# Minimap2onGPU/mm2-gb

Measured on AMD Instinct MI355X. Metric: chaining anchor-pairs/s, higher is better.
Workload: dtype int32+f32

## Files before the change

mm2-gb_amd/csrc/chain_kernels.hip:

```cpp
#include <hip/hip_runtime.h>
#include <stdint.h>
#include <limits.h>
#include <algorithm>
#include "chain_dev.h"
#include "wave_scan.h"

namespace mm2gb {

#define WAVE 64

__device__ __forceinline__ int lane_id() { return threadIdx.x & (WAVE - 1); }
__device__ __forceinline__ int bcast(int v, int src_lane) { return __builtin_amdgcn_readlane(v, src_lane); }
__device__ __forceinline__ int first_lane(int v) { return __builtin_amdgcn_readfirstlane(v); }
__device__ __forceinline__ int wave_max_i32_dpp(int v)
{
	v = max(v, __builtin_amdgcn_update_dpp(INT_MIN, v, 0x111, 0xf, 0xf, false));
	v = max(v, __builtin_amdgcn_update_dpp(INT_MIN, v, 0x112, 0xf, 0xf, false));
	v = max(v, __builtin_amdgcn_update_dpp(INT_MIN, v, 0x114, 0xf, 0xf, false));
	v = max(v, __builtin_amdgcn_update_dpp(INT_MIN, v, 0x118, 0xf, 0xf, false));
	v = max(v, __builtin_amdgcn_update_dpp(INT_MIN, v, 0x142, 0xa, 0xf, false));
	v = max(v, __builtin_amdgcn_update_dpp(INT_MIN, v, 0x143, 0xc, 0xf, false));
	return __builtin_amdgcn_readlane(v, WAVE - 1);
}
__device__ __forceinline__ int prev_lane(int v) { return __builtin_amdgcn_update_dpp(v, v, 0x138, 0xf, 0xf, false); }
// ... 540 lines not shown
			} else sc -= (int)(lin + .5f * lg);
		}
		sc_out = sc;
		return ok;
	}
}

struct Target { int x, y, tag, seg, q, st, hi; bool live; };
struct Keep { int idx, x, hi, y, tag, f; };

typedef const int __attribute__((address_space(4))) *scalar_i32_ptr;
typedef const int __attribute__((address_space(3))) *lds_i32_ptr;
__device__ __forceinline__ scalar_i32_ptr as_scalar(const void *p) { return (scalar_i32_ptr)(uintptr_t)p; }

struct SrcGroup { int x[4], y[4], t[4]; };
__device__ __forceinline__ SrcGroup load_group(const DevBatch &b, int j0)
{
	const scalar_i32_ptr sr = as_scalar(b.raw);
	SrcGroup g;
#pragma unroll
	for (int u = 0; u < 4; ++u) { const size_t at = (size_t)(j0 + u) * 4; g.x[u] = sr[at]; g.y[u] = sr[at + 2]; g.t[u] = tag_of((unsigned)sr[at + 3]); }
	return g;
}
template <bool CHECK, bool CLAMP>
__device__ __forceinline__ void sweep_block_lut(int t_st, int tx4, int ty4, int jb, int k_from, const int4 *stage,
                                                const DevParams &P, int &bestv)
{
	const unsigned base = (unsigned)P.lut_base, last_at = base + ((unsigned)P.lut_last << 2), lim4 = (unsigned)P.dq_lim << 2;
	constexpr int G = SWEEP_GROUP;
	for (int kg = k_from & ~(G - 1); kg < WAVE; kg += G) {
		const int j0 = jb + kg;
		int dqm[G], drm[G], pen[G];
		int4 s4[G];
#pragma unroll
		for (int u = 0; u < G; ++u) s4[u] = stage[kg + u];
#pragma unroll
		for (int u = 0; u < G; ++u) {
			dqm[u] = ty4 - s4[u].w; drm[u] = tx4 - s4[u].z;
			const unsigned at = lut_address(drm[u], dqm[u], base);
			pen[u] = *(lds_i32_ptr)(uintptr_t)(CLAMP ? (at < last_at ? at : last_at) : at);
		}
#pragma unroll
		for (int u = 0; u < G; ++u) {
			const int dg = drm[u] < dqm[u] ? drm[u] : dqm[u];
			int v = ((s4[u].y < dg ? s4[u].y : dg) << 5) + s4[u].x;
			asm("" : "+v"(v));
			v += pen[u];
			if (!CHECK) {
				unsigned long long saved;
				asm volatile("s_mov_b64 %[sv], exec\n\tv_cmpx_gt_u32_e32 vcc, %[lim], %[dq]\n\tv_max_i32_e32 %[b], %[v], %[b]\n\ts_mov_b64 exec, %[sv]"
				             : [b] "+v"(bestv), [sv] "=&s"(saved) : [lim] "s"(lim4), [dq] "v"(dqm[u]), [v] "v"(v) : "vcc");
			} else {
				const bool take = ((unsigned)dqm[u] < lim4) & (v > bestv) & (drm[u] != -4) & (j0 + u >= t_st);
				bestv = take ? v : bestv;
			}
		}
	}
}

template <int MODE, bool CHECK>
__device__ __forceinline__ void sweep_block(const DevBatch &b, const Target &T, int jb, int k_from, int sf,
                                            const DevParams &P, const int *lut, int &best, int &arg)
{
	int kg = k_from & ~3;
	SrcGroup nxt = load_group(b, jb + kg);
	for (; kg < WAVE; kg += 4) {
		const SrcGroup g = nxt;
		const int j0 = jb + kg;
		nxt = load_group(b, kg + 4 < WAVE ? j0 + 4 : j0);
#pragma unroll
		for (int u = 0; u < 4; ++u) {
			const int j = j0 + u;
			const int uf = bcast(sf, kg + u);
			int sc;
			bool take = pair_score<MODE>(T.x, T.y, T.seg, g.x[u], g.y[u], g.t[u], P, lut, sc);
			const int cand = sc + uf;
			take = take && cand >= best;
			if (CHECK) take = take && j >= T.st;
			if (take) { best = cand; arg = j; }
		}
	}
}

__device__ __forceinline__ void stage_block_lut(int xs, int ys, int sf, int sq, int4 *stage, bool far = false, int d0 = 0)
{
	const int k = lane_id();
	const int x4 = (int)((unsigned)xs << 2), y4 = (int)((unsigned)ys << 2);
	stage[k] = make_int4(((sf + 1) << 7) + k + 1 - LUT_BIAS + (far ? (sq - 1) << 7 : 0), far ? (int)((unsigned)(x4 - y4 - d0) ^ 0x80000000u) : (sq - 1) * 4, x4, y4);
	__builtin_amdgcn_wave_barrier();
}
__device__ __forceinline__ void stage_block_lut(const DevBatch &b, int jb, int sf, int sq, int4 *stage)
{
	const int js = jb + lane_id();
	stage_block_lut(a_x(b, js), a_y(b, js), sf, sq, stage);
}
struct TileXY { int x, y, st; };
template <bool FAR>
__device__ __forceinline__ void sweep_block_lut_free(int tx4, int ty4, const int4 *stage, const unsigned base, const int d0, int &bestv)
{
	constexpr int G = 4;
	const int td = (int)((unsigned)(tx4 - ty4 - d0) ^ 0x80000000u);
	for (int kg = 0; kg < WAVE; kg += G) {
		int4 s4[G];
		int dqm[G], drm[G], pen[G], v[G];
#pragma unroll
		for (int u = 0; u < G; ++u) {
			if (FAR) { const int2 h = *(const int2*)&stage[kg + u]; s4[u].x = h.x; s4[u].y = h.y; }
			else s4[u] = stage[kg + u];
		}
#pragma unroll
		for (int u = 0; u < G; ++u) {
			if (FAR) pen[u] = *(lds_i32_ptr)(uintptr_t)lut_address(td, s4[u].y, base);
			else {
				dqm[u] = ty4 - s4[u].w; drm[u] = tx4 - s4[u].z;
				pen[u] = *(lds_i32_ptr)(uintptr_t)lut_address(drm[u], dqm[u], base);
			}
		}
#pragma unroll
		for (int u = 0; u < G; ++u) {
			if (FAR) v[u] = s4[u].x + pen[u];
			else {
				const int dg = drm[u] < dqm[u] ? drm[u] : dqm[u];
				v[u] = ((s4[u].y < dg ? s4[u].y : dg) << 5) + s4[u].x;
				asm("" : "+v"(v[u]));
				v[u] += pen[u];
			}
		}
		asm("v_max3_i32 %0, %1, %2, %0" : "+v"(bestv) : "v"(v[0]), "v"(v[1]));
		asm("v_max3_i32 %0, %1, %2, %0" : "+v"(bestv) : "v"(v[2]), "v"(v[3]));
	}
}
__device__ __forceinline__ void sweep_block_lut_edge(int t_st, int tx4, int ty4, int jb, int k_from, const int4 *stage, const DevParams &P, int &bestv, const int k_to = WAVE)
{
	constexpr int G = 4;
	const unsigned base = (unsigned)P.lut_base, lim4 = (unsigned)P.dq_lim << 2;
	int pos = 0x7fffffff;
	asm volatile("" : "+v"(pos));
	for (int kg = k_from & ~(G - 1); kg < k_to; kg += G) {
		int4 s4[G];
		int dqm[G], drm[G], pen[G];
#pragma unroll
		for (int u = 0; u < G; ++u) s4[u] = stage[kg + u];
#pragma unroll
		for (int u = 0; u < G; ++u) {
			dqm[u] = ty4 - s4[u].w; drm[u] = tx4 - s4[u].z;
			pen[u] = *(lds_i32_ptr)(uintptr_t)lut_address(drm[u], dqm[u] & pos, base);
		}
#pragma unroll
		for (int u = 0; u < G; ++u) {
			const int dg = drm[u] < dqm[u] ? drm[u] : dqm[u];
			int v = ((s4[u].y < dg ? s4[u].y : dg) << 5) + s4[u].x;
			asm("" : "+v"(v));
			v += pen[u];
			const int j = jb + kg + u;
			unsigned long long saved;
			asm volatile("s_mov_b64 %[sv], exec\n\tv_cmpx_gt_u32_e32 vcc, %[lim], %[dq]\n\tv_cmpx_ge_i32_e32 vcc, %[j], %[st]\n\tv_max_i32_e32 %[b], %[v], %[b]\n\ts_mov_b64 exec, %[sv]"
			             : [b] "+v"(bestv), [sv] "=&s"(saved) : [lim] "s"(lim4), [dq] "v"(dqm[u]), [st] "v"(t_st), [j] "s"(j), [v] "v"(v) : "vcc");
		}
	}
}
__device__ __forceinline__ void sweep_staged_lut(const TileXY &T, int jb, int k_from, bool no_check, bool free_block, const int4 *stage, const DevParams &P,
                                                 int &best, int &arg, bool far_block = false, int d0 = 0)
{
	const int tx4 = (int)(((unsigned)T.x - 1u) << 2), ty4 = (int)(((unsigned)T.y - 1u) << 2);
	int bestv = best << 7;
	if (far_block) sweep_block_lut_free<true>(tx4, ty4, stage, (unsigned)P.lut_base, d0, bestv);
	else if (free_block) sweep_block_lut_free<false>(tx4, ty4, stage, (unsigned)P.lut_base, 0, bestv);
	else if (!no_check && !P.lut_clamp) sweep_block_lut_edge(T.st, tx4, ty4, jb, k_from, stage, P, bestv);
	else if (P.lut_clamp) {
		if (no_check) sweep_block_lut<false, true>(T.st, tx4, ty4, jb, k_from, stage, P, bestv);
		else sweep_block_lut<true, true>(T.st, tx4, ty4, jb, k_from, stage, P, bestv);
	} else {
// ... 499 lines not shown
				const int k_from = tile_lo > jb ? tile_lo - jb : 0;
				sweep_any<MODE>(b, T, jb, k_from, sf, sq, jb >= st_hi && jb + WAVE <= eq_lo, stage, P, lut, best, arg);
				sf = nf; sq = nq;
			}
		}
		in_tile<MODE, TRACK>(b, T, i0, n_here, P, lut, stage, best, arg, keep, [&](int jj) { return b.f[jj]; });
		if (T.live) {
			const int i = i0 + lane;
			b.f[i] = arg < 0 ? T.q : best;
			b.p[i] = arg < 0 ? 0 : i - arg;
		}
	}
}

struct TilePair {
	TileXY A, B;
	int n_a, n_b;
	int lo_a, hi_a, lo_b, hi_b;
	int x_first, x_last_a, x_last;
	int best_a, arg_a, best_b, arg_b;
};

__device__ __forceinline__ TileXY load_xy(const DevBatch &b, int i0, int ce, int &best)
{
	const int i = i0 + lane_id();
	const bool live = i < ce;
	const int il = live ? i : ce - 1;
	TileXY t;
	t.x = a_x(b, il); t.y = a_y(b, il);
	t.st = live ? b.st[il] : INT_MAX;
	best = a_span(b, il) + 1;
	return t;
}

__device__ __forceinline__ TilePair load_pair(const DevBatch &b, int i0, int ce)
{
	TilePair t;
	t.n_a = min(WAVE, ce - i0);
	t.n_b = max(0, min(WAVE, ce - i0 - WAVE));
	t.A = load_xy(b, i0, ce, t.best_a);
	t.B = load_xy(b, t.n_b ? i0 + WAVE : i0, ce, t.best_b);
	t.lo_a = first_lane(t.A.st); t.hi_a = bcast(t.A.st, t.n_a - 1);
	t.lo_b = t.n_b ? first_lane(t.B.st) : INT_MAX; t.hi_b = t.n_b ? bcast(t.B.st, t.n_b - 1) : INT_MAX;
	t.x_first = first_lane(t.A.x); t.x_last_a = bcast(t.A.x, t.n_a - 1);
	t.x_last = t.n_b ? bcast(t.B.x, t.n_b - 1) : t.x_last_a;
	t.arg_a = -1; t.arg_b = -1;
	return t;
}

__device__ __forceinline__ void sweep_pair_block(const DevBatch &b, TilePair &t, int jb, int eq_lo, int sf, int sq, int4 *stage, const DevParams &P)
{
	const bool nc_a = jb >= t.hi_a && jb + WAVE <= eq_lo;
	const bool use_b = t.n_b > 0 && jb + WAVE > t.lo_b;
	const bool nc_b = use_b && jb >= t.hi_b && jb + WAVE <= eq_lo;
	const int xs = a_x(b, jb + lane_id()), ys = a_y(b, jb + lane_id());
	const unsigned free_span = (unsigned)(P.dq_lim - P.bw);
	const bool free_block = P.free_sweep && (unsigned)(t.x_last - first_lane(xs)) <= free_span;
	const bool free_a = P.free_sweep && (unsigned)(t.x_last_a - first_lane(xs)) <= free_span;
	const bool single = t.n_b == 0;
	const bool far_block = free_block && nc_a && (nc_b || single) && t.x_first > bcast(xs, WAVE - 1) && __ballot(sq + P.bw > t.x_first - bcast(xs, WAVE - 1)) == 0;
	const int d0 = (first_lane(xs) - first_lane(ys)) * 4;
	stage_block_lut(xs, ys, sf, sq, stage, far_block, d0);
	if (nc_a && nc_b) sweep_staged_lut2(t.A, t.B, jb, free_block, far_block, d0, stage, P, t.best_a, t.arg_a, t.best_b, t.arg_b);
	else {
		sweep_staged_lut(t.A, jb, t.lo_a > jb ? t.lo_a - jb : 0, nc_a, nc_a && free_a, stage, P, t.best_a, t.arg_a, far_block, d0);
		if (use_b) sweep_staged_lut(t.B, jb, t.lo_b > jb ? t.lo_b - jb : 0, nc_b, nc_b && free_block, stage, P, t.best_b, t.arg_b);
	}
	__builtin_amdgcn_wave_barrier();
}

__device__ __forceinline__ void sweep_a_into_b(const DevBatch &b, TilePair &t, int cs, int i0, int f_a, int q_a, int4 *stage, const DevParams &P)
{
	if (i0 + WAVE <= t.lo_b) return;
	stage_block_lut(b, i0, f_a, q_a, stage);
	const int eq_lo = equal_x_run_start(b, cs, i0 + WAVE, first_lane(t.B.x));
	const bool no_check = i0 >= t.hi_b && i0 + WAVE <= eq_lo;
	const bool span_ab = P.free_sweep && (unsigned)(t.x_last - t.x_first) <= (unsigned)(P.dq_lim - P.bw);
	sweep_staged_lut(t.B, i0, t.lo_b > i0 ? t.lo_b - i0 : 0, no_check, no_check && span_ab, stage, P, t.best_b, t.arg_b);
	__builtin_amdgcn_wave_barrier();
}

__device__ __forceinline__ int wave_min_i32(int v) { return -wave_max_i32_dpp(-v); }

__device__ __forceinline__ void sweep_block_lut_band(int t_st, int tx4, int ty4, int idx, const int4 *stage, const DevParams &P, int &bestv)
{
	constexpr int G = 4;
	const unsigned base = (unsigned)P.lut_base, lim4 = (unsigned)P.dq_lim << 2;
	int pos = 0x7fffffff;
	asm volatile("" : "+v"(pos));
	for (int kg = 0; kg < WAVE; kg += G) {
		int4 s4[G];
		int dqm[G], drm[G], pen[G];
#pragma unroll
		for (int u = 0; u < G; ++u) s4[u] = stage[kg + u];
#pragma unroll
		for (int u = 0; u < G; ++u) {
			dqm[u] = ty4 - s4[u].w; drm[u] = tx4 - s4[u].z;
			pen[u] = *(lds_i32_ptr)(uintptr_t)lut_address(drm[u], dqm[u] & pos, base);
		}
#pragma unroll
		for (int u = 0; u < G; ++u) {
			const int dg = drm[u] < dqm[u] ? drm[u] : dqm[u];
			int v = ((s4[u].y < dg ? s4[u].y : dg) << 5) + s4[u].x;
			asm("" : "+v"(v));
			v += pen[u];
			const int j = __builtin_amdgcn_readlane(idx, kg + u);
			unsigned long long saved;
			asm volatile("s_mov_b64 %[sv], exec\n\tv_cmpx_gt_u32_e32 vcc, %[lim], %[dq]\n\tv_cmpx_ge_i32_e32 vcc, %[j], %[st]\n\tv_max_i32_e32 %[b], %[v], %[b]\n\ts_mov_b64 exec, %[sv]"
			             : [b] "+v"(bestv), [sv] "=&s"(saved) : [lim] "s"(lim4), [dq] "v"(dqm[u]), [st] "v"(t_st), [j] "s"(j), [v] "v"(v) : "vcc");
		}
	}
}

__device__ __forceinline__ int band_group(const DevBatch &b, const DevParams &P, int4 *stage, const int tgt, const int jl)
{
	const int lane = lane_id();
	const int l0 = __builtin_ctzll(__ballot(tgt >= 0));
	const int t = tgt >= 0 ? tgt : bcast(tgt, l0);
	const int x = a_x(b, t), y = a_y(b, t), st = b.st[t];
	int best = a_span(b, t) + 1, arg = -1;
	const int lo = wave_min_i32(st), hi_st = wave_max_i32_dpp(st);
	if (lo < jl) {
		const int d = x - y;
		const int dmin = wave_min_i32(d), dmax = wave_max_i32_dpp(d);
		const int gx_min = wave_min_i32(x), gx_max = wave_max_i32_dpp(x);
		const int band_lo = dmin - P.bw;
		const unsigned width = (unsigned)(dmax - dmin) + 2u * (unsigned)P.bw;
		const int tx4 = (int)(((unsigned)x - 1u) << 2), ty4 = (int)(((unsigned)y - 1u) << 2);
		const unsigned free_span = (unsigned)(P.dq_lim - P.bw);
		auto sweep = [&](const int idx) __attribute__((always_inline)) {
			const int xs = a_x(b, idx), ys = a_y(b, idx), sq = a_span(b, idx), sf = b.f[idx];
			const int sx_min = wave_min_i32(xs), sx_max = wave_max_i32_dpp(xs);
			const bool no_check = first_lane(idx) >= hi_st && gx_min > sx_max;
			const bool free_block = no_check && P.free_sweep && (unsigned)(gx_max - sx_min) <= free_span;
			const bool far_block = free_block && __ballot(sq + P.bw > gx_min - xs) == 0;
			const int d0 = (first_lane(xs) - first_lane(ys)) * 4;
			stage_block_lut(xs, ys, sf, sq, stage, far_block, d0);
			int bestv = best << 7;
			if (far_block) sweep_block_lut_free<true>(tx4, ty4, stage, (unsigned)P.lut_base, d0, bestv);
			else if (free_block) sweep_block_lut_free<false>(tx4, ty4, stage, (unsigned)P.lut_base, 0, bestv);
			else if (no_check) sweep_block_lut<false, false>(st, tx4, ty4, 0, 0, stage, P, bestv);
			else sweep_block_lut_band(st, tx4, ty4, idx, stage, P, bestv);
			const int won = bestv & 127;
			const int wj = __shfl(idx, (won - 1) & (WAVE - 1));
			arg = (unsigned)(won - 1) < (unsigned)WAVE ? wj : arg;
			best = bestv >> 7;
			__builtin_amdgcn_wave_barrier();
		};
		int sidx = 0, n_st = 0;
		int jb = lo;
		int dn = jb + lane < jl ? __hip_atomic_load(b.diag + jb + lane, __ATOMIC_RELAXED, __HIP_MEMORY_SCOPE_AGENT) : 0;
		for (; jb < jl; jb += WAVE) {
			const int j = jb + lane;
			const int dj = dn;
			dn = j + WAVE < jl ? __hip_atomic_load(b.diag + j + WAVE, __ATOMIC_RELAXED, __HIP_MEMORY_SCOPE_AGENT) : 0;
			const bool hit = j < jl && (unsigned)(dj - band_lo) <= width;
			const unsigned long long m = __ballot(hit);
			if (m == 0) continue;
			const int c = __popcll(m);
			const int rank = __builtin_amdgcn_mbcnt_hi((unsigned)(m >> 32), __builtin_amdgcn_mbcnt_lo((unsigned)m, 0u));
			const int dst = (hit ? n_st + rank : n_st + c) & (WAVE - 1);
			const int recv = __builtin_amdgcn_ds_permute(dst << 2, j);
			if (n_st + c < WAVE) {
				sidx = lane >= n_st && lane < n_st + c ? recv : sidx;
				n_st += c;
			} else {
				sweep(lane >= n_st ? recv : sidx);
				n_st += c - WAVE;
				sidx = recv;
			}
		}
		if (n_st > 0) sweep(lane < n_st ? sidx : bcast(sidx, n_st - 1));
	}
	if (tgt >= 0) { b.band_res[2 * tgt] = best; b.band_res[2 * tgt + 1] = arg; }
	return lo < jl;
}

__device__ __forceinline__ int band_slab_part(const DevBatch &b, const DevParams &P, int4 *stage, const int s0, const int n, const int jl,
                                              const int g_from, const int g_to)
{
	constexpr int R = 8;
	const int lane = lane_id();
	unsigned key[R];
	int lo = INT_MAX, hi = INT_MIN, st_lo = INT_MAX;
#pragma unroll
	for (int r = 0; r < R; ++r) {
		const int e = r * WAVE + lane;
		const int d = e < n ? a_x(b, s0 + e) - a_y(b, s0 + e) : 0;
		if (e < n) { lo = min(lo, d); hi = max(hi, d); st_lo = min(st_lo, b.st[s0 + e]); }
	}
	if (wave_min_i32(st_lo) >= jl) return 0;
	const int dmin = wave_min_i32(lo), dmax = wave_max_i32_dpp(hi);
	const unsigned range = (unsigned)(dmax - dmin);
	if (range <= 2u * (unsigned)P.bw) {
#pragma unroll
		for (int r = 0; r < R; ++r) key[r] = r * WAVE + lane < n ? (unsigned)(r * WAVE + lane) : ~0u;
	} else {
		const int sh = (range >> 22) ? 32 - __clz((int)(range >> 22)) : 0;
#pragma unroll
		for (int r = 0; r < R; ++r) {
			const int e = r * WAVE + lane;
			key[r] = e < n ? (((unsigned)(a_x(b, s0 + e) - a_y(b, s0 + e) - dmin) >> sh) << 9) | (unsigned)e : ~0u;
		}
#pragma unroll
		for (int k = 2; k <= R * WAVE; k <<= 1) {
#pragma unroll
			for (int j = k >> 1; j > 0; j >>= 1) {
				if (j >= WAVE) {
					const int jr = j / WAVE;
#pragma unroll
					for (int r = 0; r < R; ++r) {
						if (r & jr) continue;
						const bool up = ((r * WAVE) & k) == 0;
						const unsigned a = key[r], c = key[r | jr];
						key[r] = up ? min(a, c) : max(a, c);
						key[r | jr] = up ? max(a, c) : min(a, c);
					}
				} else {
#pragma unroll
					for (int r = 0; r < R; ++r) {
						const unsigned o = (unsigned)__shfl_xor((int)key[r], j);
						const bool up = ((r * WAVE + lane) & k) == 0, lower = (lane & j) == 0;
						key[r] = up == lower ? min(key[r], o) : max(key[r], o);
					}
				}
			}
		}
	}
	int swept = 0;
	for (int g = g_from; g < g_to; ++g) {
		unsigned kg = key[0];
#pragma unroll
		for (int r = 1; r < R; ++r) kg = g == r ? key[r] : kg;
		const int tgt = kg == ~0u ? -1 : s0 + (int)(kg & 511u);
		if (__ballot(tgt >= 0) == 0) break;
		swept += band_group(b, P, stage, tgt, jl);
	}
	return swept;
}
__device__ __forceinline__ bool band_fits_team(const DevParams &P, const int anchors_per_part, const int n_waves)
{
	return P.band_slab > 0 && P.band_slab / anchors_per_part <= n_waves;
}
__device__ __forceinline__ bool band_chunk(const DevBatch &b, const DevParams &P, const int ci, const int cs, const int ce)
{
	const long long len = ce - cs;
	return P.band_slab > 0 && b.band_res && 2 * (b.chunk_cost[ci] - 16 * len) > (long long)P.band_lag * len;
}

__device__ __forceinline__ void band_merge(const DevBatch &b, const int i0, const int n_here, int &best, int &arg)
{
	const int i = i0 + min(lane_id(), n_here - 1);
	const int bb = __hip_atomic_load(b.band_res + 2 * i, __ATOMIC_RELAXED, __HIP_MEMORY_SCOPE_AGENT);
	const int ba = __hip_atomic_load(b.band_res + 2 * i + 1, __ATOMIC_RELAXED, __HIP_MEMORY_SCOPE_AGENT);
	const bool take = ba >= 0 && (arg < 0 || bb > best);
	best = take ? bb : best;
	arg = take ? ba : arg;
}

__device__ __forceinline__ void band_store_diag(const DevBatch &b, const TilePair &t, const int i0)
{
	if (lane_id() < t.n_a) b.diag[i0 + lane_id()] = t.A.x - t.A.y;
	if (lane_id() < t.n_b) b.diag[i0 + WAVE + lane_id()] = t.B.x - t.B.y;
}

template <bool TRACK>
__device__ __forceinline__ void run_chunk_pairs(const DevBatch &b, const DevParams &P, const int *lut, int4 *stage, const int cs, const int ce, const bool band_on)
{
	const int lane = lane_id();
	Keep keep; keep.idx = -1; keep.x = keep.hi = keep.y = keep.tag = keep.f = 0;
	auto f_old = [&](int jj) { return b.f[jj]; };
	const bool band = band_on;
	int band_groups = 0;
	for (int i0 = cs; i0 < ce; i0 += 2 * WAVE) {
		TilePair t = load_pair(b, i0, ce);
		int jb = cs + ((t.lo_a - cs) & ~(WAVE - 1));
		const int s0 = band ? i0 - (i0 - cs) % P.band_slab : cs, jl = s0 - P.band_lag;
		const bool in_band = band && jl > cs;
		if (band) band_store_diag(b, t, i0);
		if (in_band && i0 == s0) {
			band_groups += band_slab_part(b, P, stage, s0, min(P.band_slab, ce - s0), jl, 0, P.band_slab / WAVE);
			asm volatile("s_waitcnt vmcnt(0)" ::: "memory");
		}
		if (in_band && jb < jl) jb = jl;
		if (jb < i0) {
			const int eq_lo = equal_x_run_start(b, cs, i0, first_lane(t.A.x));
			int sf = b.f[jb + lane], sq = a_span(b, jb + lane);
			for (; jb < i0; jb += WAVE) {
				const int jn = jb + WAVE < i0 ? jb + WAVE + lane : jb + lane;
				const int nf = b.f[jn], nq = a_span(b, jn);
				sweep_pair_block(b, t, jb, eq_lo, sf, sq, stage, P);
				sf = nf; sq = nq;
			}
		}
		const Target TA = load_target(b, i0, ce, TRACK);
		if (in_band && t.lo_a < jl) band_merge(b, i0, t.n_a, t.best_a, t.arg_a);
		in_tile<MODE_LUT, TRACK>(b, TA, i0, t.n_a, P, lut, stage, t.best_a, t.arg_a, keep, f_old);
		const int f_a = t.arg_a < 0 ? TA.q : t.best_a;
		if (TA.live) {
			const int i = i0 + lane;
			b.f[i] = f_a;
			b.p[i] = t.arg_a < 0 ? 0 : i - t.arg_a;
		}
		if (t.n_b == 0) break;
		sweep_a_into_b(b, t, cs, i0, f_a, TA.q, stage, P);
		const Target TB = load_target(b, i0 + WAVE, ce, TRACK);
		if (in_band && t.lo_b < jl) band_merge(b, i0 + WAVE, t.n_b, t.best_b, t.arg_b);
		in_tile<MODE_LUT, TRACK>(b, TB, i0 + WAVE, t.n_b, P, lut, stage, t.best_b, t.arg_b, keep, f_old);
		if (TB.live) {
			const int i = i0 + WAVE + lane;
			b.f[i] = t.arg_b < 0 ? TB.q : t.best_b;
			b.p[i] = t.arg_b < 0 ? 0 : i - t.arg_b;
		}
	}
	if (band_groups > 0 && lane == 0) atomicAdd(&b.counters[CNT_BAND_WAVE], band_groups);
}

struct CoopShared { int done; int keep[6]; int chunk; int bar_count; int bar_gen; int part; int band; };
#define MM2GB_AGENT __HIP_MEMORY_SCOPE_AGENT
__device__ __forceinline__ int  gload(const int *p) { return __hip_atomic_load(p, __ATOMIC_RELAXED, MM2GB_AGENT); }
__device__ __forceinline__ void gstore(int *p, int v) { __hip_atomic_store(p, v, __ATOMIC_RELAXED, MM2GB_AGENT); }
__device__ __forceinline__ void drain_stores() { asm volatile("s_waitcnt vmcnt(0)" ::: "memory"); }
constexpr int SMALL_TEAM = 4, N_SMALL_TEAMS = SCORE_THREADS / WAVE / SMALL_TEAM;
constexpr int N_TEAM_RECORDS = N_SMALL_TEAMS + 3;
constexpr int TAB_INTS = 12;

__device__ __forceinline__ void team_barrier(CoopShared *sh, int team_size)
{
	__builtin_amdgcn_fence(__ATOMIC_RELEASE, "workgroup");
	if (lane_id() == 0) {
		const int gen = __hip_atomic_load(&sh->bar_gen, __ATOMIC_RELAXED, __HIP_MEMORY_SCOPE_WORKGROUP);
		if (__hip_atomic_fetch_add(&sh->bar_count, 1, __ATOMIC_ACQ_REL, __HIP_MEMORY_SCOPE_WORKGROUP) == team_size - 1) {
			__hip_atomic_store(&sh->bar_count, 0, __ATOMIC_RELAXED, __HIP_MEMORY_SCOPE_WORKGROUP);
			__hip_atomic_fetch_add(&sh->bar_gen, 1, __ATOMIC_RELEASE, __HIP_MEMORY_SCOPE_WORKGROUP);
		} else {
			while (__hip_atomic_load(&sh->bar_gen, __ATOMIC_ACQUIRE, __HIP_MEMORY_SCOPE_WORKGROUP) == gen) __builtin_amdgcn_s_sleep(2);
		}
	}
	__builtin_amdgcn_fence(__ATOMIC_ACQUIRE, "workgroup");
}

template <class TT, class SF, class WQ>
__device__ __forceinline__ void sweep_block_by_quarters(const DevBatch &b, const TT &T, const int jb, const int k_from, const int sq, int4 *stage, const DevParams &P,
                                                        int &best, int &arg, SF &&sf_of, WQ &&wait_q)
{
	const int xs = a_x(b, jb + lane_id()), ys = a_y(b, jb + lane_id());
	const int tx4 = (int)(((unsigned)T.x - 1u) << 2), ty4 = (int)(((unsigned)T.y - 1u) << 2);
	for (int q = 0; q < 4; ++q) {
		wait_q(q);
		const int lo = max(k_from, 16 * q), hi = 16 * q + 16;
		if (lo >= hi) continue;
		stage_block_lut(xs, ys, sf_of(), sq, stage);
		int bestv = best << 7;
		sweep_block_lut_edge(T.st, tx4, ty4, jb, lo, stage, P, bestv, hi);
		const int won = bestv & 127;
		arg = (unsigned)(won - 1) < (unsigned)WAVE ? jb + won - 1 : arg;
		best = bestv >> 7;
		__builtin_amdgcn_wave_barrier();
	}
}

template <int MODE, bool TRACK>
__device__ __forceinline__ void coop_chunk(const DevBatch &b, const DevParams &P, const int *lut, int4 *stage, int *ring, const int n_slots, CoopShared *sh,
                           const int cs, const int ce, const int wave, const int n_waves, const bool band_on)
{
	const int lane = lane_id();
	const int n_tiles = (ce - cs + WAVE - 1) / WAVE;
	auto wait_done = [&](int need) {
		while (first_lane(__hip_atomic_load(&sh->done, __ATOMIC_ACQUIRE, __HIP_MEMORY_SCOPE_WORKGROUP)) < need) __builtin_amdgcn_s_sleep(MM2GB_POLL_SLEEP);
	};
	const bool band = MODE == MODE_LUT && band_on && band_fits_team(P, WAVE, n_waves);
	const int tps = band ? P.band_slab / WAVE : 1, s_first = band ? P.band_lag / P.band_slab + 1 : 0;
	int band_groups = 0;
	for (int t = wave; t < n_tiles; t += n_waves) {
		const int i0 = cs + t * WAVE;
		const Target T = load_target(b, i0, ce, TRACK);
		const int n_here = min(WAVE, ce - i0);
		int best = T.q + 1, arg = -1;
		const int tile_lo = first_lane(T.st);
		const int st_hi = bcast(T.st, n_here - 1);
		int jb = cs + ((tile_lo - cs) & ~(WAVE - 1));
		const int sl = t / tps, s0 = cs + sl * P.band_slab, jl = s0 - P.band_lag;
		const bool in_band = band && jl > cs;
		int *band_cnt = sl & 1 ? &sh->band : &sh->part;
		if (band && T.live) b.diag[i0 + lane] = T.x - T.y;
		if (in_band) {
			const int part = t - sl * tps;
			wait_done((jl - cs) / WAVE);
			band_groups += band_slab_part(b, P, stage, s0, min(P.band_slab, ce - s0), jl, part, part + 1);
			if (lane == 0) __hip_atomic_fetch_add(band_cnt, 1, __ATOMIC_RELEASE, __HIP_MEMORY_SCOPE_WORKGROUP);
			if (jb < jl) jb = jl;
		}
		const int eq_lo = MODE == MODE_LUT && jb < i0 ? equal_x_run_start(b, cs, i0, first_lane(T.x)) : i0;
		int slot = (int)((unsigned)((jb - cs) / WAVE) % (unsigned)n_slots);
		for (; jb < i0; jb += WAVE) {
			const int sq = MODE == MODE_LUT ? a_span(b, jb + lane) : 0;
			const int k = (jb - cs) / WAVE, k_from = tile_lo > jb ? tile_lo - jb : 0;
			wait_done(k + 1);
			const int sf = ring[slot * WAVE + lane];
			slot = slot + 1 == n_slots ? 0 : slot + 1;
			sweep_any<MODE>(b, T, jb, k_from, sf, sq, jb >= st_hi && jb + WAVE <= eq_lo, stage, P, lut, best, arg);
		}
		const int my_slot = (int)((unsigned)t % (unsigned)n_slots);
		wait_done(t);
		if (in_band && tile_lo < jl) {
			const int s_min = s_first + ((sl - s_first) & 1);
			const int need = tps * ((sl - s_min) / 2) + min(tps, n_tiles - sl * tps);
			while (first_lane(__hip_atomic_load(band_cnt, __ATOMIC_ACQUIRE, __HIP_MEMORY_SCOPE_WORKGROUP)) < need) __builtin_amdgcn_s_sleep(MM2GB_POLL_SLEEP);
			band_merge(b, i0, n_here, best, arg);
		}
		Keep keep;
		if (TRACK) { keep.idx = first_lane(sh->keep[0]); keep.x = first_lane(sh->keep[1]); keep.hi = first_lane(sh->keep[2]); keep.y = first_lane(sh->keep[3]); keep.tag = first_lane(sh->keep[4]); keep.f = first_lane(sh->keep[5]); }
		else { keep.idx = -1; keep.x = keep.hi = keep.y = keep.tag = keep.f = 0; }
		in_tile<MODE, TRACK>(b, T, i0, n_here, P, lut, stage, best, arg, keep,
		                     [&](int jj) { const unsigned d = (unsigned)(jj - cs); return ring[(d / WAVE) % (unsigned)n_slots * WAVE + d % WAVE]; });
		const int i = i0 + lane;
		const int fi = arg < 0 ? T.q : best;
		if (T.live) {
			ring[my_slot * WAVE + lane] = fi;
			b.f[i] = fi;
			b.p[i] = arg < 0 ? 0 : i - arg;
		}
		if (TRACK && lane == 0) { sh->keep[0] = keep.idx; sh->keep[1] = keep.x; sh->keep[2] = keep.hi; sh->keep[3] = keep.y; sh->keep[4] = keep.tag; sh->keep[5] = keep.f; }
		if (lane == 0) __hip_atomic_store(&sh->done, t + 1, __ATOMIC_RELEASE, __HIP_MEMORY_SCOPE_WORKGROUP);
	}
	if (band_groups > 0 && lane == 0) atomicAdd(&b.counters[CNT_BAND_TEAM], band_groups);
}

template <bool TRACK>
__device__ __forceinline__ void coop_chunk_pairs(const DevBatch &b, const DevParams &P, const int *lut, int4 *stage, int *ring, const int n_slots, CoopShared *sh,
                                 const int cs, const int ce, const int wave, const int n_waves, const bool band_on)
{
	const int lane = lane_id();
	const int n_tiles = (ce - cs + WAVE - 1) / WAVE;
	auto wait_done = [&](int need) {
		while (first_lane(__hip_atomic_load(&sh->done, __ATOMIC_ACQUIRE, __HIP_MEMORY_SCOPE_WORKGROUP)) < need) __builtin_amdgcn_s_sleep(MM2GB_POLL_SLEEP);
	};
	int cur = 0;
	const lds_i32_ptr ring_l = (lds_i32_ptr)(uintptr_t)(unsigned)(uintptr_t)ring;
	auto f_old = [&](int jj) {
		const unsigned d = (unsigned)(jj - cs);
		const int k = (int)(d / WAVE);
		return k >= cur - n_slots ? ring_l[(unsigned)k % (unsigned)n_slots * WAVE + d % WAVE] : b.f[jj];
	};
	const bool band = band_on && band_fits_team(P, 2 * WAVE, n_waves);
	const int pps = band ? P.band_slab / (2 * WAVE) : 1, n_pairs = (n_tiles + 1) / 2, s_first = band ? P.band_lag / P.band_slab + 1 : 0;
	int band_groups = 0;
	for (int pr = wave; 2 * pr < n_tiles; pr += n_waves) {
		const int ta = 2 * pr, i0 = cs + ta * WAVE;
		TilePair t = load_pair(b, i0, ce);
		int jb = cs + ((t.lo_a - cs) & ~(WAVE - 1));
		const int sl = pr / pps, s0 = cs + sl * P.band_slab, jl = s0 - P.band_lag;
		const bool in_band = band && jl > cs;
		int *band_cnt = sl & 1 ? &sh->band : &sh->part;
		if (band) band_store_diag(b, t, i0);
		if (in_band) {
			const int part = pr - sl * pps;
			wait_done((jl - cs) / WAVE);
			band_groups += band_slab_part(b, P, stage, s0, min(P.band_slab, ce - s0), jl, 2 * part, 2 * part + 2);
			if (lane == 0) __hip_atomic_fetch_add(band_cnt, 1, __ATOMIC_RELEASE, __HIP_MEMORY_SCOPE_WORKGROUP);
			if (jb < jl) jb = jl;
		}
		const int eq_lo = jb < i0 ? equal_x_run_start(b, cs, i0, first_lane(t.A.x)) : i0;
		int slot = (int)((unsigned)((jb - cs) / WAVE) % (unsigned)n_slots);
		const int first_in_ring = ta - n_slots;
		int nf = 0;
		if (jb < i0 && (jb - cs) / WAVE < first_in_ring) { wait_done((jb - cs) / WAVE + 1); nf = b.f[jb + lane]; }
		for (; jb < i0; jb += WAVE) {
			const int sq = a_span(b, jb + lane);
			const int k = (jb - cs) / WAVE;
			wait_done(k + 1);
			int sf;
			if (k < first_in_ring) {
				sf = nf;
				if (k + 1 < first_in_ring) { wait_done(k + 2); nf = b.f[jb + WAVE + lane]; }
			} else sf = ring[slot * WAVE + lane];
			slot = slot + 1 == n_slots ? 0 : slot + 1;
			sweep_pair_block(b, t, jb, eq_lo, sf, sq, stage, P);
		}
		const int slot_a = (int)((unsigned)ta % (unsigned)n_slots), slot_b = slot_a + 1 == n_slots ? 0 : slot_a + 1;
		wait_done(ta);
		Keep keep;
		if (TRACK) { keep.idx = first_lane(sh->keep[0]); keep.x = first_lane(sh->keep[1]); keep.hi = first_lane(sh->keep[2]); keep.y = first_lane(sh->keep[3]); keep.tag = first_lane(sh->keep[4]); keep.f = first_lane(sh->keep[5]); }
		else { keep.idx = -1; keep.x = keep.hi = keep.y = keep.tag = keep.f = 0; }
		const Target TA = load_target(b, i0, ce, TRACK);
		if (in_band && t.lo_a < jl) {
			const int s_min = s_first + ((sl - s_first) & 1);
			const int need = pps * ((sl - s_min) / 2) + min(pps, n_pairs - sl * pps);
			while (first_lane(__hip_atomic_load(band_cnt, __ATOMIC_ACQUIRE, __HIP_MEMORY_SCOPE_WORKGROUP)) < need) __builtin_amdgcn_s_sleep(MM2GB_POLL_SLEEP);
			band_merge(b, i0, t.n_a, t.best_a, t.arg_a);
		}
		cur = ta;
		in_tile<MODE_LUT, TRACK>(b, TA, i0, t.n_a, P, lut, stage, t.best_a, t.arg_a, keep, f_old);
		__builtin_amdgcn_s_setprio(MM2GB_INTILE_PRIO);
		const int f_a = t.arg_a < 0 ? TA.q : t.best_a;
		if (TA.live) {
			const int i = i0 + lane;
			ring[slot_a * WAVE + lane] = f_a;
			b.f[i] = f_a;
			b.p[i] = t.arg_a < 0 ? 0 : i - t.arg_a;
		}
		if (t.n_b > 0) {
			if (lane == 0) __hip_atomic_store(&sh->done, ta + 1, __ATOMIC_RELEASE, __HIP_MEMORY_SCOPE_WORKGROUP);
			sweep_a_into_b(b, t, cs, i0, f_a, TA.q, stage, P);
			const Target TB = load_target(b, i0 + WAVE, ce, TRACK);
			if (in_band && t.lo_b < jl) {
				const int s_min = s_first + ((sl - s_first) & 1);
				const int need = pps * ((sl - s_min) / 2) + min(pps, n_pairs - sl * pps);
				while (first_lane(__hip_atomic_load(band_cnt, __ATOMIC_ACQUIRE, __HIP_MEMORY_SCOPE_WORKGROUP)) < need) __builtin_amdgcn_s_sleep(MM2GB_POLL_SLEEP);
				band_merge(b, i0 + WAVE, t.n_b, t.best_b, t.arg_b);
			}
			cur = ta + 1;
			in_tile<MODE_LUT, TRACK>(b, TB, i0 + WAVE, t.n_b, P, lut, stage, t.best_b, t.arg_b, keep, f_old);
			__builtin_amdgcn_s_setprio(MM2GB_INTILE_PRIO);
			if (TB.live) {
				const int i = i0 + WAVE + lane;
				const int f_b = t.arg_b < 0 ? TB.q : t.best_b;
				ring[slot_b * WAVE + lane] = f_b;
				b.f[i] = f_b;
				b.p[i] = t.arg_b < 0 ? 0 : i - t.arg_b;
			}
		}
		if (TRACK && lane == 0) { sh->keep[0] = keep.idx; sh->keep[1] = keep.x; sh->keep[2] = keep.hi; sh->keep[3] = keep.y; sh->keep[4] = keep.tag; sh->keep[5] = keep.f; }
		if (lane == 0) __hip_atomic_store(&sh->done, ta + (t.n_b > 0 ? 2 : 1), __ATOMIC_RELEASE, __HIP_MEMORY_SCOPE_WORKGROUP);
		__builtin_amdgcn_s_setprio(0);
	}
	if (band_groups > 0 && lane == 0) atomicAdd(&b.counters[CNT_BAND_TEAM], band_groups);
}


template <bool TRACK>
__device__ __forceinline__ void gang_chunk_pairs(const DevBatch &b, const DevParams &P, const int *lut, int4 *stage, int *ring, const int n_slots, CoopShared *sh,
                                 GangSlot *gs, int *tab, int &seq, const int cs, const int ce, const int wave)
{
	const int lane = lane_id();
	const int n_tiles = (ce - cs + WAVE - 1) / WAVE;
	const int tpu = first_lane(gload(&gs->tiles_per_wave)) == 2 ? 2 : 1;
	const int STRIP_TILES = tpu * GANG_STRIP_PAIRS;
	int known = 0, known_global = 0;
	auto look_global = [&]() { known_global = max(known_global, first_lane(gload(&gs->done))); known = max(known, known_global); };
	auto wait_done = [&](int need) {
		if (known >= need) return;
		for (;;) {
			known = max(known, first_lane(__hip_atomic_load(&sh->done, __ATOMIC_ACQUIRE, __HIP_MEMORY_SCOPE_WORKGROUP)));
			if (known >= need) return;
// ... 437 lines not shown
```

profiles/isa_loops.py:

```python
#!/usr/bin/env python3
import collections, os, re, subprocess, sys, tempfile
ROOT = os.path.dirname(os.path.dirname(os.path.abspath(__file__)))
SRC = os.path.join(ROOT, "mm2-gb_amd", "csrc", os.environ.get("MM2GB_ISA_SRC", "chain_kernels.hip"))
want = sys.argv[1] if len(sys.argv) > 1 else "k_scoreILi0ELb0ELb0E"
min_len = int(sys.argv[2]) if len(sys.argv) > 2 else 6
HALF = re.compile(r"^v_(sad_u32|min3|max3|lshl_add|add3|and_or|min_|max_|cmp|cmpx|readlane|readfirstlane|writelane|cvt_|mul_lo|mul_hi|mad_|bfe|perm|lshl_or|or3|xad|add_lshl|med3)")

with tempfile.TemporaryDirectory() as td:
    asm = os.path.join(td, "k.s")
    subprocess.run(["/opt/rocm/bin/hipcc", "--offload-arch=gfx950", "-O3", "-std=c++17", "-fPIC", "-ffp-contract=off", "-gline-tables-only", "-I" + os.path.join(ROOT, "include"),
                    "--cuda-device-only", "-S", SRC, "-o", asm], check=True, stderr=subprocess.DEVNULL)
    lines = open(asm).read().splitlines()

src = open(SRC).read().splitlines()
fn_at = []
for i, ln in enumerate(src, 1):
    m = re.match(r"^(?:template\s*<[^>]*>\s*)?(?:static\s+)?(?:__device__|__global__)[^()]*?\b([A-Za-z_][A-Za-z0-9_]*)\s*\(", ln)
    if m:
        fn_at.append((i, m.group(1)))
    else:
        m = re.match(r"^\s+__device__ __forceinline__ [^()]*?\b([A-Za-z_][A-Za-z0-9_]*)\s*\(", ln)
        if m:
            fn_at.append((i, m.group(1)))


def fn_of(line):
    name = "?"
    for at, n in fn_at:
        if at <= line:
            name = n
        else:
            break
    return name


start = next(i for i, ln in enumerate(lines) if ln.startswith("_ZN5mm2gb") and want in ln and ln.rstrip().split(":")[0].endswith(ln.split(":")[0]) and ":" in ln)
end = next(i for i in range(start, len(lines)) if lines[i].startswith(".Lfunc_end"))
file_ids = {}
for ln in lines:
    m = re.match(r'\s*\.file\s+(\d+)\s+"([^"]*)"(?:\s+"([^"]*)")?', ln)
    if m:
        file_ids[int(m.group(1))] = (m.group(3) or m.group(2))
body = []
labels = {}
cur = (0, False)
for i in range(start + 1, end):
    ln = lines[i]
    m = re.match(r"\s*\.loc\s+(\d+)\s+(\d+)", ln)
    if m:
        cur = (int(m.group(2)), file_ids.get(int(m.group(1)), "").endswith(os.path.basename(SRC)))
        continue
    m = re.match(r"^(\.LBB\d+_\d+):", ln)
    if m:
        labels[m.group(1)] = len(body)
        continue
    t = ln.strip()
    if not t or t.startswith(";") or t.startswith("."):
        continue
    body.append((t.split()[0], t, cur[0] if cur[1] else 0))

reg_users = collections.defaultdict(set)
for op, text, _ in body:
    for r in re.findall(r"\bv(\d+)\b", text):
        reg_users[int(r)].add(op)
spill_vgprs = {r for r, ops in reg_users.items() if "v_writelane_b32" in ops and ops <= {"v_writelane_b32", "v_readlane_b32"}}


def is_spill(o):
    if "Spill" in o[1] or "Reload" in o[1] or o[0].startswith("scratch_"):
        return True
    if o[0] == "v_writelane_b32":
        m = re.match(r"v_writelane_b32 v(\d+)", o[1]); return bool(m) and int(m.group(1)) in spill_vgprs
    if o[0] == "v_readlane_b32":
        m = re.match(r"v_readlane_b32 s\d+, v(\d+)", o[1]); return bool(m) and int(m.group(1)) in spill_vgprs
    return False


def mix(ops):
    valu = [o for o in ops if o[0].startswith("v_") and not is_spill(o)]
    return {"n": len(ops), "valu": len(valu), "half": sum(1 for o in valu if HALF.match(o[0])),
            "salu": sum(1 for o in ops if o[0].startswith("s_") and not o[0].startswith(("s_waitcnt", "s_nop"))),
            "lds": sum(1 for o in ops if o[0].startswith("ds_")), "mem": sum(1 for o in ops if o[0].startswith(("global_", "buffer_", "flat_"))),
            "wait": sum(1 for o in ops if o[0].startswith("s_waitcnt")), "spill": sum(1 for o in ops if is_spill(o)),
            "bread": sum(1 for o in ops if o[0] in ("ds_read_b128", "ds_read2_b64", "ds_read_b64") )}


fn_ranges = []
# ... 52 lines not shown
```

Before: 7008 billion.

## Outline band slab pass into noinline function with address-space-typed uniform arguments

Turns band_slab_part into a __noinline__ function. Its arguments are raw address_space(1)/(3) pointers plus scalar params, re-made uniform with readfirstlane. The sweep lambda is folded into a single while loop, the diag key is reused instead of reloading x/y, and the band pass now runs before the tile loads in each driver loop. The aim is to cut register pressure and spills in the main scoring loops by keeping the band code's registers separate. In exchange it adds call overhead and changes the ordering of the band pass relative to the diag stores.

Measured after the change: 7245 billion, median of 6. 3.4% higher.

```diff
diff --git a/mm2-gb_amd/csrc/chain_kernels.hip b/mm2-gb_amd/csrc/chain_kernels.hip
--- a/mm2-gb_amd/csrc/chain_kernels.hip
+++ b/mm2-gb_amd/csrc/chain_kernels.hip
@@ -646,12 +646,15 @@
 	}
 }
 
-__device__ __forceinline__ void stage_block_lut(int xs, int ys, int sf, int sq, int4 *stage, bool far = false, int d0 = 0)
-{
-	const int k = lane_id();
+__device__ __forceinline__ void stage_block_lut_at(const int k, int xs, int ys, int sf, int sq, int4 *stage, bool far = false, int d0 = 0)
+{
 	const int x4 = (int)((unsigned)xs << 2), y4 = (int)((unsigned)ys << 2);
 	stage[k] = make_int4(((sf + 1) << 7) + k + 1 - LUT_BIAS + (far ? (sq - 1) << 7 : 0), far ? (int)((unsigned)(x4 - y4 - d0) ^ 0x80000000u) : (sq - 1) * 4, x4, y4);
 	__builtin_amdgcn_wave_barrier();
+}
+__device__ __forceinline__ void stage_block_lut(int xs, int ys, int sf, int sq, int4 *stage, bool far = false, int d0 = 0)
+{
+	stage_block_lut_at(lane_id(), xs, ys, sf, sq, stage, far, d0);
 }
 __device__ __forceinline__ void stage_block_lut(const DevBatch &b, int jb, int sf, int sq, int4 *stage)
 {
@@ -1317,6 +1320,20 @@
 
 __device__ __forceinline__ int wave_min_i32(int v) { return -wave_max_i32_dpp(-v); }
 
+typedef const int __attribute__((address_space(1))) *glb_i32_cptr;
+typedef int __attribute__((address_space(1))) *glb_i32_ptr;
+typedef int4 __attribute__((address_space(3))) *lds_i32x4_ptr;
+__device__ __forceinline__ int lane_by_count() { return (int)__builtin_amdgcn_mbcnt_hi(~0u, __builtin_amdgcn_mbcnt_lo(~0u, 0u)); }
+struct BandParams { int bw, dq_lim, lut_base, free_sweep, band_slab; };
+template <class T> __device__ __forceinline__ T uniform_glb(T p)
+{
+	const unsigned long long v = (unsigned long long)(uintptr_t)p;
+	return (T)(uintptr_t)(((unsigned long long)(unsigned)first_lane((int)(v >> 32)) << 32) | (unsigned)first_lane((int)v));
+}
+__device__ __forceinline__ int r_x(glb_i32_cptr raw, int i) { return raw[(size_t)i * 4]; }
+__device__ __forceinline__ int r_y(glb_i32_cptr raw, int i) { return raw[(size_t)i * 4 + 2]; }
+__device__ __forceinline__ int r_span(glb_i32_cptr raw, int i) { return (int)((unsigned)raw[(size_t)i * 4 + 3] & 0xffu); }
+
 __device__ __forceinline__ void sweep_block_lut_band(int t_st, int tx4, int ty4, int idx, const int4 *stage, const DevParams &P, int &bestv)
 {
 	constexpr int G = 4;
@@ -1347,13 +1364,15 @@
 	}
 }
 
-__device__ __forceinline__ int band_group(const DevBatch &b, const DevParams &P, int4 *stage, const int tgt, const int jl)
-{
-	const int lane = lane_id();
+struct BandIO { glb_i32_cptr raw, st, f, diag; glb_i32_ptr res; };
+
+__device__ __forceinline__ int band_group(const BandIO &b, const DevParams &P, int4 *stage, const int tgt, const int jl)
+{
+	const int lane = lane_by_count();
 	const int l0 = __builtin_ctzll(__ballot(tgt >= 0));
 	const int t = tgt >= 0 ? tgt : bcast(tgt, l0);
-	const int x = a_x(b, t), y = a_y(b, t), st = b.st[t];
-	int best = a_span(b, t) + 1, arg = -1;
+	const int x = r_x(b.raw, t), y = r_y(b.raw, t), st = b.st[t];
+	int best = r_span(b.raw, t) + 1, arg = -1;
 	const int lo = wave_min_i32(st), hi_st = wave_max_i32_dpp(st);
 	if (lo < jl) {
 		const int d = x - y;
@@ -1363,14 +1382,42 @@
 		const unsigned width = (unsigned)(dmax - dmin) + 2u * (unsigned)P.bw;
 		const int tx4 = (int)(((unsigned)x - 1u) << 2), ty4 = (int)(((unsigned)y - 1u) << 2);
 		const unsigned free_span = (unsigned)(P.dq_lim - P.bw);
-		auto sweep = [&](const int idx) __attribute__((always_inline)) {
-			const int xs = a_x(b, idx), ys = a_y(b, idx), sq = a_span(b, idx), sf = b.f[idx];
+		int sidx = 0, n_st = 0;
+		int jb = lo;
+		int dn = jb + lane < jl ? __hip_atomic_load(b.diag + jb + lane, __ATOMIC_RELAXED, __HIP_MEMORY_SCOPE_AGENT) : 0;
+		while (true) {
+			int idx, carry = 0, n_next = 0;
+			if (jb < jl) {
+				const int j = jb + lane;
+				const int dj = dn;
+				dn = j + WAVE < jl ? __hip_atomic_load(b.diag + j + WAVE, __ATOMIC_RELAXED, __HIP_MEMORY_SCOPE_AGENT) : 0;
+				jb += WAVE;
+				const bool hit = j < jl && (unsigned)(dj - band_lo) <= width;
+				const unsigned long long m = __ballot(hit);
+				if (m == 0) continue;
+				const int c = __popcll(m);
+				const int rank = __builtin_amdgcn_mbcnt_hi((unsigned)(m >> 32), __builtin_amdgcn_mbcnt_lo((unsigned)m, 0u));
+				const int dst = (hit ? n_st + rank : n_st + c) & (WAVE - 1);
+				const int recv = __builtin_amdgcn_ds_permute(dst << 2, j);
+				if (n_st + c < WAVE) {
+					sidx = lane >= n_st && lane < n_st + c ? recv : sidx;
+					n_st += c;
+					continue;
+				}
+				idx = lane >= n_st ? recv : sidx;
+				n_next = n_st + c - WAVE;
+				carry = recv;
+			} else {
+				if (n_st == 0) break;
+				idx = lane < n_st ? sidx : bcast(sidx, n_st - 1);
+			}
+			const int xs = r_x(b.raw, idx), ys = r_y(b.raw, idx), sq = r_span(b.raw, idx), sf = b.f[idx];
 			const int sx_min = wave_min_i32(xs), sx_max = wave_max_i32_dpp(xs);
 			const bool no_check = first_lane(idx) >= hi_st && gx_min > sx_max;
 			const bool free_block = no_check && P.free_sweep && (unsigned)(gx_max - sx_min) <= free_span;
 			const bool far_block = free_block && __ballot(sq + P.bw > gx_min - xs) == 0;
 			const int d0 = (first_lane(xs) - first_lane(ys)) * 4;
-			stage_block_lut(xs, ys, sf, sq, stage, far_block, d0);
+			stage_block_lut_at(lane, xs, ys, sf, sq, stage, far_block, d0);
 			int bestv = best << 7;
 			if (far_block) sweep_block_lut_free<true>(tx4, ty4, stage, (unsigned)P.lut_base, d0, bestv);
 			else if (free_block) sweep_block_lut_free<false>(tx4, ty4, stage, (unsigned)P.lut_base, 0, bestv);
@@ -1381,47 +1428,31 @@
 			arg = (unsigned)(won - 1) < (unsigned)WAVE ? wj : arg;
 			best = bestv >> 7;
 			__builtin_amdgcn_wave_barrier();
-		};
-		int sidx = 0, n_st = 0;
-		int jb = lo;
-		int dn = jb + lane < jl ? __hip_atomic_load(b.diag + jb + lane, __ATOMIC_RELAXED, __HIP_MEMORY_SCOPE_AGENT) : 0;
-		for (; jb < jl; jb += WAVE) {
-			const int j = jb + lane;
-			const int dj = dn;
-			dn = j + WAVE < jl ? __hip_atomic_load(b.diag + j + WAVE, __ATOMIC_RELAXED, __HIP_MEMORY_SCOPE_AGENT) : 0;
-			const bool hit = j < jl && (unsigned)(dj - band_lo) <= width;
-			const unsigned long long m = __ballot(hit);
-			if (m == 0) continue;
-			const int c = __popcll(m);
-			const int rank = __builtin_amdgcn_mbcnt_hi((unsigned)(m >> 32), __builtin_amdgcn_mbcnt_lo((unsigned)m, 0u));
-			const int dst = (hit ? n_st + rank : n_st + c) & (WAVE - 1);
-			const int recv = __builtin_amdgcn_ds_permute(dst << 2, j);
-			if (n_st + c < WAVE) {
-				sidx = lane >= n_st && lane < n_st + c ? recv : sidx;
-				n_st += c;
-			} else {
-				sweep(lane >= n_st ? recv : sidx);
-				n_st += c - WAVE;
-				sidx = recv;
-			}
-		}
-		if (n_st > 0) sweep(lane < n_st ? sidx : bcast(sidx, n_st - 1));
-	}
-	if (tgt >= 0) { b.band_res[2 * tgt] = best; b.band_res[2 * tgt + 1] = arg; }
+			sidx = carry; n_st = n_next;
+		}
+	}
+	if (tgt >= 0) { b.res[2 * tgt] = best; b.res[2 * tgt + 1] = arg; }
 	return lo < jl;
 }
 
-__device__ __forceinline__ int band_slab_part(const DevBatch &b, const DevParams &P, int4 *stage, const int s0, const int n, const int jl,
-                                              const int g_from, const int g_to)
+__device__ __noinline__ int band_slab_part(const glb_i32_cptr raw_, const glb_i32_cptr st_, const glb_i32_cptr f_, const glb_i32_cptr diag_, const glb_i32_ptr res_,
+                                           const BandParams bp, const lds_i32x4_ptr stage_, const int s0_, const int ce_, const int jl_, const int g_from_, const int g_to_)
 {
 	constexpr int R = 8;
-	const int lane = lane_id();
+	const BandIO b = { uniform_glb(raw_), uniform_glb(st_), uniform_glb(f_), uniform_glb(diag_), uniform_glb(res_) };
+	DevParams P = {};
+	P.bw = first_lane(bp.bw); P.dq_lim = first_lane(bp.dq_lim); P.lut_base = first_lane(bp.lut_base); P.free_sweep = first_lane(bp.free_sweep);
+	int4 *stage = (int4*)(lds_i32x4_ptr)(uintptr_t)(unsigned)first_lane((int)(unsigned)(uintptr_t)stage_);
+	const int s0 = first_lane(s0_), jl = first_lane(jl_), g_from = first_lane(g_from_), g_to = first_lane(g_to_);
+	const int n = min(first_lane(bp.band_slab), first_lane(ce_) - s0);
+	const int lane = lane_by_count();
 	unsigned key[R];
 	int lo = INT_MAX, hi = INT_MIN, st_lo = INT_MAX;
 #pragma unroll
 	for (int r = 0; r < R; ++r) {
 		const int e = r * WAVE + lane;
-		const int d = e < n ? a_x(b, s0 + e) - a_y(b, s0 + e) : 0;
+		const int d = e < n ? r_x(b.raw, s0 + e) - r_y(b.raw, s0 + e) : 0;
+		key[r] = (unsigned)d;
 		if (e < n) { lo = min(lo, d); hi = max(hi, d); st_lo = min(st_lo, b.st[s0 + e]); }
 	}
 	if (wave_min_i32(st_lo) >= jl) return 0;
@@ -1435,7 +1466,7 @@
 #pragma unroll
 		for (int r = 0; r < R; ++r) {
 			const int e = r * WAVE + lane;
-			key[r] = e < n ? (((unsigned)(a_x(b, s0 + e) - a_y(b, s0 + e) - dmin) >> sh) << 9) | (unsigned)e : ~0u;
+			key[r] = e < n ? (((unsigned)((int)key[r] - dmin) >> sh) << 9) | (unsigned)e : ~0u;
 		}
 #pragma unroll
 		for (int k = 2; k <= R * WAVE; k <<= 1) {
@@ -1473,6 +1504,12 @@
 	}
 	return swept;
 }
+__device__ __forceinline__ int band_pass(const DevBatch &b, const DevParams &P, int4 *stage, const int s0, const int ce, const int jl, const int g_from, const int g_to)
+{
+	const BandParams bp = { P.bw, P.dq_lim, P.lut_base, P.free_sweep, P.band_slab };
+	return first_lane(band_slab_part((glb_i32_cptr)(const int*)b.raw, (glb_i32_cptr)b.st, (glb_i32_cptr)b.f, (glb_i32_cptr)b.diag, (glb_i32_ptr)b.band_res,
+	                                 bp, (lds_i32x4_ptr)stage, s0, ce, jl, g_from, g_to));
+}
 __device__ __forceinline__ bool band_fits_team(const DevParams &P, const int anchors_per_part, const int n_waves)
 {
 	return P.band_slab > 0 && P.band_slab / anchors_per_part <= n_waves;
@@ -1508,15 +1545,15 @@
 	const bool band = band_on;
 	int band_groups = 0;
 	for (int i0 = cs; i0 < ce; i0 += 2 * WAVE) {
+		const int s0 = band ? i0 - (i0 - cs) % P.band_slab : cs, jl = s0 - P.band_lag;
+		const bool in_band = band && jl > cs;
+		if (in_band && i0 == s0) {
+			band_groups += band_pass(b, P, stage, s0, ce, jl, 0, P.band_slab / WAVE);
+			asm volatile("s_waitcnt vmcnt(0)" ::: "memory");
+		}
 		TilePair t = load_pair(b, i0, ce);
 		int jb = cs + ((t.lo_a - cs) & ~(WAVE - 1));
-		const int s0 = band ? i0 - (i0 - cs) % P.band_slab : cs, jl = s0 - P.band_lag;
-		const bool in_band = band && jl > cs;
 		if (band) band_store_diag(b, t, i0);
-		if (in_band && i0 == s0) {
-			band_groups += band_slab_part(b, P, stage, s0, min(P.band_slab, ce - s0), jl, 0, P.band_slab / WAVE);
-			asm volatile("s_waitcnt vmcnt(0)" ::: "memory");
-		}
 		if (in_band && jb < jl) jb = jl;
 		if (jb < i0) {
 			const int eq_lo = equal_x_run_start(b, cs, i0, first_lane(t.A.x));
@@ -1609,23 +1646,23 @@
 	int band_groups = 0;
 	for (int t = wave; t < n_tiles; t += n_waves) {
 		const int i0 = cs + t * WAVE;
+		const int sl = t / tps, s0 = cs + sl * P.band_slab, jl = s0 - P.band_lag;
+		const bool in_band = band && jl > cs;
+		int *band_cnt = sl & 1 ? &sh->band : &sh->part;
+		if (in_band) {
+			const int part = t - sl * tps;
+			wait_done((jl - cs) / WAVE);
+			band_groups += band_pass(b, P, stage, s0, ce, jl, part, part + 1);
+			if (lane == 0) __hip_atomic_fetch_add(band_cnt, 1, __ATOMIC_RELEASE, __HIP_MEMORY_SCOPE_WORKGROUP);
+		}
 		const Target T = load_target(b, i0, ce, TRACK);
 		const int n_here = min(WAVE, ce - i0);
 		int best = T.q + 1, arg = -1;
 		const int tile_lo = first_lane(T.st);
 		const int st_hi = bcast(T.st, n_here - 1);
 		int jb = cs + ((tile_lo - cs) & ~(WAVE - 1));
-		const int sl = t / tps, s0 = cs + sl * P.band_slab, jl = s0 - P.band_lag;
-		const bool in_band = band && jl > cs;
-		int *band_cnt = sl & 1 ? &sh->band : &sh->part;
 		if (band && T.live) b.diag[i0 + lane] = T.x - T.y;
-		if (in_band) {
-			const int part = t - sl * tps;
-			wait_done((jl - cs) / WAVE);
-			band_groups += band_slab_part(b, P, stage, s0, min(P.band_slab, ce - s0), jl, part, part + 1);
-			if (lane == 0) __hip_atomic_fetch_add(band_cnt, 1, __ATOMIC_RELEASE, __HIP_MEMORY_SCOPE_WORKGROUP);
-			if (jb < jl) jb = jl;
-		}
+		if (in_band && jb < jl) jb = jl;
 		const int eq_lo = MODE == MODE_LUT && jb < i0 ? equal_x_run_start(b, cs, i0, first_lane(T.x)) : i0;
 		int slot = (int)((unsigned)((jb - cs) / WAVE) % (unsigned)n_slots);
 		for (; jb < i0; jb += WAVE) {
@@ -1683,19 +1720,19 @@
 	int band_groups = 0;
 	for (int pr = wave; 2 * pr < n_tiles; pr += n_waves) {
 		const int ta = 2 * pr, i0 = cs + ta * WAVE;
-		TilePair t = load_pair(b, i0, ce);
-		int jb = cs + ((t.lo_a - cs) & ~(WAVE - 1));
 		const int sl = pr / pps, s0 = cs + sl * P.band_slab, jl = s0 - P.band_lag;
 		const bool in_band = band && jl > cs;
 		int *band_cnt = sl & 1 ? &sh->band : &sh->part;
-		if (band) band_store_diag(b, t, i0);
 		if (in_band) {
 			const int part = pr - sl * pps;
 			wait_done((jl - cs) / WAVE);
-			band_groups += band_slab_part(b, P, stage, s0, min(P.band_slab, ce - s0), jl, 2 * part, 2 * part + 2);
+			band_groups += band_pass(b, P, stage, s0, ce, jl, 2 * part, 2 * part + 2);
 			if (lane == 0) __hip_atomic_fetch_add(band_cnt, 1, __ATOMIC_RELEASE, __HIP_MEMORY_SCOPE_WORKGROUP);
-			if (jb < jl) jb = jl;
-		}
+		}
+		TilePair t = load_pair(b, i0, ce);
+		int jb = cs + ((t.lo_a - cs) & ~(WAVE - 1));
+		if (band) band_store_diag(b, t, i0);
+		if (in_band && jb < jl) jb = jl;
 		const int eq_lo = jb < i0 ? equal_x_run_start(b, cs, i0, first_lane(t.A.x)) : i0;
 		int slot = (int)((unsigned)((jb - cs) / WAVE) % (unsigned)n_slots);
 		const int first_in_ring = ta - n_slots;
diff --git a/profiles/isa_loops.py b/profiles/isa_loops.py
--- a/profiles/isa_loops.py
+++ b/profiles/isa_loops.py
@@ -2,7 +2,7 @@
 import collections, os, re, subprocess, sys, tempfile
 ROOT = os.path.dirname(os.path.dirname(os.path.abspath(__file__)))
 SRC = os.path.join(ROOT, "mm2-gb_amd", "csrc", os.environ.get("MM2GB_ISA_SRC", "chain_kernels.hip"))
-want = sys.argv[1] if len(sys.argv) > 1 else "k_scoreILi0ELb0ELb0E"
+want = sys.argv[1] if len(sys.argv) > 1 else "k_scoreILi0ELb0EE"
 min_len = int(sys.argv[2]) if len(sys.argv) > 2 else 6
 HALF = re.compile(r"^v_(sad_u32|min3|max3|lshl_add|add3|and_or|min_|max_|cmp|cmpx|readlane|readfirstlane|writelane|cvt_|mul_lo|mul_hi|mad_|bfe|perm|lshl_or|or3|xad|add_lshl|med3)")
 
```
